# wanmeihuali/taichi_3d_gaussian_splatting

Hardware: NVIDIA H100
Metric: rendered Mpix/sec fwd+bwd @1080p, 1e6 Gaussians (higher is better)
Workload: dtype f32

## Files before the change

### taichi_3d_gaussian_splatting_b200/csrc/blend_bwd_transposed.cu

```cuda
#include "blend_bwd.cuh"

namespace gsb {

constexpr int TB_CHUNK = 16;
constexpr int TB_ROW = TB_CHUNK + 1;
constexpr int TB_TR_ROW = 13;

struct TbShared {
    float4 rec[2 * 3 * GSB_TILE_PIXELS];
    float4 g[8][32];
    float xg[8][32 * TB_ROW];
    float xa[8][32 * TB_ROW];
    int off[2][GSB_TILE_PIXELS];
    float4 chunk[8][3][TB_CHUNK];
    int chunk_off[8][TB_CHUNK];
    unsigned int bits[2][8][8];
    unsigned char list[8][GSB_TILE_PIXELS];
    int max_last;
};
static_assert(32 * TB_ROW >= TB_CHUNK * TB_TR_ROW, "finished rows must fit into the exchange buffer");

#ifdef GSB_HOST_EMU
static inline unsigned char *tb_dynamic_smem() { return simt_emu::dynamic_smem(); }
#else
extern __shared__ __align__(16) unsigned char gsb_tb_dynamic_smem[];
__device__ __forceinline__ unsigned char *tb_dynamic_smem() { return gsb_tb_dynamic_smem; }
#endif

#ifndef GSB_TB_P1_UNROLL
#define GSB_TB_P1_UNROLL 4
#endif
constexpr int TB_P1_UNROLL = GSB_TB_P1_UNROLL;
#ifndef GSB_TB_MIN_BLOCKS
#define GSB_TB_MIN_BLOCKS 3
#endif
__device__ __forceinline__ float keep_if_contributing(float P, int idx, int last) {
#ifdef GSB_HOST_EMU
    return ((idx < last) && (P >= 1.0f / 255.0f)) ? P : 0.0f;
#else
    float r;
    asm("{\n"
        ".reg .pred p, q;\n"
        "setp.lt.s32 q, %2, %3;\n"
        "setp.ge.and.f32 p, %1, 0f3B808081, q;\n"
        "selp.f32 %0, %1, 0f00000000, p;\n"
        "}\n"
        : "=f"(r)
        : "f"(P), "r"(idx), "r"(last));
    return r;
#endif
}

template <bool EXACT_EXP, bool STATS, bool COUNT = false>
__global__ void __launch_bounds__(GSB_TILE_PIXELS, GSB_TB_MIN_BLOCKS)
blend_backward_transposed_kernel(const BlendBwdParams p) {
    TbShared &S = *reinterpret_cast<TbShared *>(tb_dynamic_smem());
    constexpr int NV = STATS ? 11 : 9;

    const int tile = blockIdx.x;
    const int tu = tile % p.tiles_x, tv = tile / p.tiles_x;
    const int tid = threadIdx.x, lane = tid & 31, warp = tid >> 5;
    const int pu = tu * GSB_TILE_WIDTH + (warp & 1) * 8 + (lane & 7);
    const int pv = tv * GSB_TILE_HEIGHT + (warp >> 1) * 4 + (lane >> 3);
    const float px = (float)pu + 0.5f, py = (float)pv + 0.5f;
    const float tile_x0 = (float)(tu * GSB_TILE_WIDTH), tile_y0 = (float)(tv * GSB_TILE_HEIGHT);
    const size_t pix = (size_t)pv * p.W + pu;
    const int start = p.tile_start[tile];

    const int last = p.last_effective[pix];
    float T = 1.0f - p.acc_alpha[pix];
    float w0 = 0.0f, w1 = 0.0f, w2 = 0.0f;
    const float g0 = p.grad_image[3 * pix], g1 = p.grad_image[3 * pix + 1], g2 = p.grad_image[3 * pix + 2];
    float mag0 = 0.0f, mag1 = 0.0f;
    unsigned int n_visits = 0, n_pairs = 0;
    S.g[warp][lane] = make_float4(g0, g1, g2, 0.0f);

    const int ci = lane & (TB_CHUNK - 1), half = lane >> 4;
    const float pxb = tile_x0 + (float)((warp & 1) * 8) + 0.5f;
    const float pyb = tile_y0 + (float)((warp >> 1) * 4 + 2 * half) + 0.5f;
    float *const xg = S.xg[warp], *const xa = S.xa[warp];
    const int fl_row = lane >= GSB_ACCUM_FLOATS ? 1 : 0;
    const int fl_word = lane - GSB_ACCUM_FLOATS * fl_row;
    const bool fl_ok = lane < 2 * GSB_ACCUM_FLOATS && fl_word < NV;
    const int *const fl_off = S.chunk_off[warp] + fl_row;
    const float *const fl_val = xg + fl_row * TB_TR_ROW + (fl_ok ? fl_word : 0);
    unsigned char *const list = S.list[warp];

    int warp_last = last;
#pragma unroll
    for (int d = 16; d > 0; d >>= 1) warp_last = max(warp_last, __shfl_xor_sync(0xffffffffu, warp_last, d));
    if (tid == 0) S.max_last = start;
    __syncthreads();
    if (lane == 0) atomicMax(&S.max_last, warp_last);
    __syncthreads();
    const int end = min(p.tile_end[tile], S.max_last);

    float4 *const ck0 = S.chunk[warp][0], *const ck1 = S.chunk[warp][1], *const ck2 = S.chunk[warp][2];
    int *const ck_off = S.chunk_off[warp];
    int have = 0;

    int buf = 0;
    for (int block_end = end;; block_end -= GSB_TILE_PIXELS, buf ^= 1) {
        const bool real = block_end > start;
        int count = 0;
        float4 *const s_r0 = S.rec + buf * 3 * GSB_TILE_PIXELS;
        float4 *const s_r1 = s_r0 + GSB_TILE_PIXELS, *const s_r2 = s_r0 + 2 * GSB_TILE_PIXELS;
        if (real) {
            const int block_start = max(block_end - GSB_TILE_PIXELS, start);
            {
                const int idx = block_end - 1 - tid;
                unsigned int mask = 0;
                if (idx >= block_start) {
                    const int o = __ldg(&p.sorted_vals[idx]);
                    const float4 *rec = p.records + 3 * (size_t)o;
                    const float4 r0 = __ldg(rec), r1 = __ldg(rec + 1);
                    if (EXACT_EXP) {
                        s_r0[tid] = r0;
                        s_r1[tid] = r1;
                    } else {
                        float4 f0, f1;
                        fast_planes(r0, r1, f0, f1);
                        s_r0[tid] = f0;
                        s_r1[tid] = f1;
                    }
                    s_r2[tid] = __ldg(rec + 2);
                    S.off[buf][tid] = o;
                    mask = splat_patch_mask(r0.x, r0.y, r0.z, r0.w, r1.x, r1.y * r1.z, tile_x0, tile_y0);
                }
#pragma unroll
                for (int w = 0; w < 8; ++w) {
                    const unsigned int bits = __ballot_sync(0xffffffffu, (mask >> w) & 1u);
                    if (lane == 0) S.bits[buf][w][warp] = bits;
                }
            }
            __syncthreads();
            if (tid == 0) GSB_EMU_COUNT(EC_BATCHES, 1);
            if (block_start < warp_last) {
                const int skip = block_end - warp_last;
#pragma unroll
                for (int k = 0; k < 8; ++k) {
                    unsigned int bits = S.bits[buf][warp][k];
                    const int lo = skip - 32 * k;
                    if (lo >= 32) bits = 0u;
                    else if (lo > 0) bits &= ~((1u << lo) - 1u);
                    if ((bits >> lane) & 1u)
                        list[count + __popc(bits & ((1u << lane) - 1u))] = (unsigned char)(k * 32 + lane);
                    count += __popc(bits);
                }
                __syncwarp();
            }
        }

        int pos = 0;
#pragma unroll 1
        do {
            if (pos < count) {
                const int take = min(TB_CHUNK - have, count - pos);
                if (lane < take) {
                    const int j = list[pos + lane], slot = have + lane;
                    ck0[slot] = s_r0[j];
                    ck1[slot] = s_r1[j];
                    float4 r2 = s_r2[j];
                    r2.w = __int_as_float(block_end - 1 - j);
                    ck2[slot] = r2;
                    ck_off[slot] = S.off[buf][j];
                }
                have += take;
                pos += take;
                __syncwarp();
            }
            if (have == TB_CHUNK || (!real && have > 0)) {
                const int n = have;
                have = 0;
                if (COUNT) n_visits += (lane == 0) ? (unsigned int)n : 0u;
                if (lane == 0) {
                    GSB_EMU_COUNT(EC_TB_SPLATS, n);
                    GSB_EMU_COUNT(EC_TB_CHUNKS, 1);
                }
#pragma unroll TB_P1_UNROLL
                for (int i = 0; i < n; ++i) {
                    const float4 r0 = ck0[i];
                    const float4 r1 = ck1[i];
                    const float4 r2 = ck2[i];
                    const int idx = __float_as_int(r2.w);
                    const float d0 = px - r0.x, d1 = py - r0.y;
                    float G, aT;
                    if (EXACT_EXP) {
                        const float q0 = r0.z * d0 + r0.w * d1;
                        const float q1 = r0.w * d0 + r1.x * d1;
                        const float gp = expf(-0.5f * (d0 * q0 + d1 * q1)) * r1.y;
                        const float prod_alpha = gp * r1.z;
                        const bool contributes = (idx < last) && (prod_alpha >= 1.0f / 255.0f);
                        const float alpha = fminf(prod_alpha, 0.99f);
                        const float inv = 1.0f / (1.0f - alpha);
                        const float Tn = T * inv;
                        aT = contributes ? alpha * Tn : 0.0f;
                        const float a_grad = contributes ? (r2.x * Tn - w0 * inv) * g0 + (r2.y * Tn - w1 * inv) * g1 +
                                                               (r2.z * Tn - w2 * inv) * g2
                                                         : 0.0f;
                        T = contributes ? Tn : T;
                        w0 = fmaf(r2.x, aT, w0);
                        w1 = fmaf(r2.y, aT, w1);
                        w2 = fmaf(r2.z, aT, w2);
                        G = a_grad * r1.z * gp;
                        if (STATS) {
                            mag0 += fabsf(G * q0);
                            mag1 += fabsf(G * q1);
                        }
                    } else {
                        float P = fast_alpha(d0, d1, r0.z, r0.w, r1.x, r1.y);
                        P = keep_if_contributing(P, idx, last);
                        const float alpha = fminf(P, 0.99f);
                        const float inv = rcp_approx(1.0f - alpha);
                        T *= inv;
                        aT = alpha * T;
                        const float cg = fmaf(r2.z, g2, fmaf(r2.y, g1, r2.x * g0));
                        const float a_grad = fmaf(cg, T, -(w0 * inv));
                        w0 = fmaf(cg, aT, w0);
                        G = a_grad * P;
                        if (STATS) {
                            const float q0 = (-2.0f / GSB_L2E) * fmaf(r0.z, d0, 0.5f * r0.w * d1);
                            const float q1 = (-2.0f / GSB_L2E) * fmaf(0.5f * r0.w, d0, r1.x * d1);
                            mag0 += fabsf(G * q0);
                            mag1 += fabsf(G * q1);
                        }
                    }
                    if (COUNT) n_pairs += aT > 0.0f ? 1u : 0u;
                    xg[lane * TB_ROW + i] = G;
                    xa[lane * TB_ROW + i] = aT;
                }
                __syncwarp();

                const bool active = ci < n;
                float4 s0 = ck0[active ? ci : 0];
                float4 s1 = ck1[active ? ci : 0];
                if (!EXACT_EXP) {
                    s0.z *= -2.0f / GSB_L2E;
                    s0.w *= -1.0f / GSB_L2E;
                    s1.x *= -2.0f / GSB_L2E;
                }
                const float dx0 = pxb - s0.x;
                float acc[11];
#pragma unroll
                for (int k = 0; k < 11; ++k) acc[k] = 0.0f;
                unsigned int nz = 0u;
#pragma unroll
                for (int row = 0; row < 2; ++row) {
                    const float d1 = (pyb + (float)row) - s0.y;
                    float q0 = s0.z * dx0 + s0.w * d1;
                    float q1 = s0.w * dx0 + s1.x * d1;
#pragma unroll
                    for (int k = 0; k < 8; ++k) {
                        const int pp = 8 * row + k + 16 * half;
                        const float G = xg[pp * TB_ROW + ci], aT = xa[pp * TB_ROW + ci];
                        const float4 gp = S.g[warp][pp];
                        const float vs0 = G * q0, vs1 = G * q1;
                        acc[0] += vs0;
                        acc[1] += vs1;
                        acc[2] = fmaf(vs0, q0, acc[2]);
                        acc[3] = fmaf(vs0, q1, acc[3]);
                        acc[4] = fmaf(vs1, q1, acc[4]);
                        acc[5] = fmaf(aT, gp.x, acc[5]);
                        acc[6] = fmaf(aT, gp.y, acc[6]);
                        acc[7] = fmaf(aT, gp.z, acc[7]);
                        acc[8] += G;
                        if (STATS) {
                            const float m2 = vs0 * vs0 + vs1 * vs1;
                            acc[9] += EXACT_EXP ? sqrtf(m2) : sqrt_approx(m2);
                            acc[10] += aT > 0.0f ? 1.0f : 0.0f;
                        }
                        nz |= __float_as_uint(aT);
                        q0 += s0.z;
                        q1 += s0.w;
                    }
                }
#pragma unroll
                for (int k = 0; k < NV; ++k) acc[k] += __shfl_xor_sync(0xffffffffu, acc[k], 16);
                nz |= __shfl_xor_sync(0xffffffffu, nz, 16);
                acc[8] *= EXACT_EXP ? (1.0f - s1.z) : s1.z;
                __syncwarp();
                if (lane < TB_CHUNK) {
                    if (!(active && nz != 0u)) ck_off[ci] = -1;
                    else GSB_EMU_COUNT(EC_TB_ROWS, 1);
#pragma unroll
                    for (int k = 0; k < NV; ++k) xg[ci * TB_TR_ROW + k] = acc[k];
                }
                __syncwarp();
#pragma unroll
                for (int step = 0; step < TB_CHUNK / 2; ++step) {
                    const int o = fl_off[2 * step];
                    const float v = fl_val[2 * step * TB_TR_ROW];
                    if (fl_ok && o >= 0) atomicAdd(p.accum + (size_t)o * GSB_ACCUM_FLOATS + fl_word, v);
                }
                __syncwarp();
            }
        } while (pos < count);
        if (!real) break;
    }
    if (STATS) {
        p.mag_image[2 * pix] = mag0;
        p.mag_image[2 * pix + 1] = mag1;
    }
    if (COUNT) {
#pragma unroll
        for (int d = 16; d > 0; d >>= 1) {
            n_visits += __shfl_xor_sync(0xffffffffu, n_visits, d);
            n_pairs += __shfl_xor_sync(0xffffffffu, n_pairs, d);
        }
        if (lane == 0) {
            atomicAdd(p.work_counters, (unsigned long long)n_visits);
            atomicAdd(p.work_counters + 1, (unsigned long long)n_pairs);
        }
    }
}

#ifndef GSB_HOST_EMU
template <bool EXACT_EXP, bool STATS>
static int launch_tb(const BlendBwdParams &p, int tiles, cudaStream_t stream) {
    static bool configured = false;
    if (!configured) {
        GSB_CUDA_CHECK(cudaFuncSetAttribute(blend_backward_transposed_kernel<EXACT_EXP, STATS>,
                                            cudaFuncAttributeMaxDynamicSharedMemorySize, (int)sizeof(TbShared)));
        configured = true;
    }
    blend_backward_transposed_kernel<EXACT_EXP, STATS><<<tiles, GSB_TILE_PIXELS, sizeof(TbShared), stream>>>(p);
    GSB_CUDA_CHECK(cudaGetLastError());
    return GSB_OK;
}

int launch_blend_backward_transposed(const BlendBwdParams &p, int tiles, bool exact_exp, bool stats,
                                     cudaStream_t stream) {
    if (exact_exp) return stats ? launch_tb<true, true>(p, tiles, stream) : launch_tb<true, false>(p, tiles, stream);
    return stats ? launch_tb<false, true>(p, tiles, stream) : launch_tb<false, false>(p, tiles, stream);
}

int launch_blend_backward_count(const BlendBwdParams &p, int tiles, cudaStream_t stream) {
    GSB_CUDA_CHECK(cudaFuncSetAttribute(blend_backward_transposed_kernel<false, false, true>,
                                        cudaFuncAttributeMaxDynamicSharedMemorySize, (int)sizeof(TbShared)));
    blend_backward_transposed_kernel<false, false, true><<<tiles, GSB_TILE_PIXELS, sizeof(TbShared), stream>>>(p);
    GSB_CUDA_CHECK(cudaGetLastError());
    return GSB_OK;
}
#endif

}
```

Measured before the change: 1153.

## Factor phase-2 moments per row, interleave G/aT, and use float4 vector atomics

Phase 2 now accumulates per-row moments (sum G, sum k*G, sum k^2*G) of the Gaussian weight and reconstructs the five geometric gradient terms algebraically per row, instead of doing per-pixel q0/q1 products. G and aT are stored interleaved as float2, and the Gaussian id is packed into r2.w so the separate offset array goes away. Per-warp shared state is regrouped into a struct. The final flush uses float4 atomicAdd (sm_90 vector reduction) over three 16-byte segments per Gaussian instead of scalar atomics. The chunk size becomes configurable (8 or 16), and phase 1 is unrolled in fixed groups for full chunks. The moment-based reconstruction changes floating-point rounding slightly, and the 12-float writes add one unused zero per row.

```diff
diff --git a/taichi_3d_gaussian_splatting_b200/csrc/blend_bwd_transposed.cu b/taichi_3d_gaussian_splatting_b200/csrc/blend_bwd_transposed.cu
--- a/taichi_3d_gaussian_splatting_b200/csrc/blend_bwd_transposed.cu
+++ b/taichi_3d_gaussian_splatting_b200/csrc/blend_bwd_transposed.cu
@@ -2,23 +2,39 @@
 
 namespace gsb {
 
-constexpr int TB_CHUNK = 16;
+#ifndef GSB_TB_CHUNK
+#define GSB_TB_CHUNK 16
+#endif
+#ifndef GSB_TB_MIN_BLOCKS
+#if GSB_TB_CHUNK == 8
+#define GSB_TB_MIN_BLOCKS 4
+#else
+#define GSB_TB_MIN_BLOCKS 3
+#endif
+#endif
+constexpr int TB_CHUNK = GSB_TB_CHUNK;
+static_assert(TB_CHUNK == 8 || TB_CHUNK == 16, "a phase-2 lane takes whole rows of the 8 x 4 patch");
+constexpr int TB_ROWS = TB_CHUNK / 8;
 constexpr int TB_ROW = TB_CHUNK + 1;
-constexpr int TB_TR_ROW = 13;
-
+
+struct TbWarp {
+    float4 g[32];
+    float4 chunk[3][TB_CHUNK];
+    float2 x[32 * TB_ROW];
+    int chunk_off[TB_CHUNK];
+    unsigned char list[GSB_TILE_PIXELS];
+};
 struct TbShared {
     float4 rec[2 * 3 * GSB_TILE_PIXELS];
-    float4 g[8][32];
-    float xg[8][32 * TB_ROW];
-    float xa[8][32 * TB_ROW];
-    int off[2][GSB_TILE_PIXELS];
-    float4 chunk[8][3][TB_CHUNK];
-    int chunk_off[8][TB_CHUNK];
+    TbWarp w[8];
     unsigned int bits[2][8][8];
-    unsigned char list[8][GSB_TILE_PIXELS];
+    float2 origin;
     int max_last;
 };
-static_assert(32 * TB_ROW >= TB_CHUNK * TB_TR_ROW, "finished rows must fit into the exchange buffer");
+static_assert(2 * 32 * TB_ROW >= TB_CHUNK * GSB_ACCUM_FLOATS && GSB_ACCUM_FLOATS == 12,
+              "the finished rows (3 float4 each) must fit into the exchange buffer");
+static_assert(GSB_TB_MIN_BLOCKS * (sizeof(TbShared) + 1024) <= 228 * 1024,
+              "the shared-memory image does not allow GSB_TB_MIN_BLOCKS CTAs per SM");
 
 #ifdef GSB_HOST_EMU
 static inline unsigned char *tb_dynamic_smem() { return simt_emu::dynamic_smem(); }
@@ -31,9 +47,17 @@
 #define GSB_TB_P1_UNROLL 4
 #endif
 constexpr int TB_P1_UNROLL = GSB_TB_P1_UNROLL;
-#ifndef GSB_TB_MIN_BLOCKS
-#define GSB_TB_MIN_BLOCKS 3
-#endif
+static_assert(TB_CHUNK % TB_P1_UNROLL == 0, "a full chunk is a whole number of phase-1 groups");
+__device__ __forceinline__ void red_add_f32x4(float *addr, const float4 v) {
+#ifdef GSB_HOST_EMU
+    atomicAdd(addr, v.x);
+    atomicAdd(addr + 1, v.y);
+    atomicAdd(addr + 2, v.z);
+    atomicAdd(addr + 3, v.w);
+#else
+    atomicAdd(reinterpret_cast<float4 *>(addr), v);
+#endif
+}
 __device__ __forceinline__ float keep_if_contributing(float P, int idx, int last) {
 #ifdef GSB_HOST_EMU
     return ((idx < last) && (P >= 1.0f / 255.0f)) ? P : 0.0f;
@@ -63,7 +87,6 @@
     const int pu = tu * GSB_TILE_WIDTH + (warp & 1) * 8 + (lane & 7);
     const int pv = tv * GSB_TILE_HEIGHT + (warp >> 1) * 4 + (lane >> 3);
     const float px = (float)pu + 0.5f, py = (float)pv + 0.5f;
-    const float tile_x0 = (float)(tu * GSB_TILE_WIDTH), tile_y0 = (float)(tv * GSB_TILE_HEIGHT);
     const size_t pix = (size_t)pv * p.W + pu;
     const int start = p.tile_start[tile];
 
@@ -73,30 +96,28 @@
     const float g0 = p.grad_image[3 * pix], g1 = p.grad_image[3 * pix + 1], g2 = p.grad_image[3 * pix + 2];
     float mag0 = 0.0f, mag1 = 0.0f;
     unsigned int n_visits = 0, n_pairs = 0;
-    S.g[warp][lane] = make_float4(g0, g1, g2, 0.0f);
-
-    const int ci = lane & (TB_CHUNK - 1), half = lane >> 4;
-    const float pxb = tile_x0 + (float)((warp & 1) * 8) + 0.5f;
-    const float pyb = tile_y0 + (float)((warp >> 1) * 4 + 2 * half) + 0.5f;
-    float *const xg = S.xg[warp], *const xa = S.xa[warp];
-    const int fl_row = lane >= GSB_ACCUM_FLOATS ? 1 : 0;
-    const int fl_word = lane - GSB_ACCUM_FLOATS * fl_row;
-    const bool fl_ok = lane < 2 * GSB_ACCUM_FLOATS && fl_word < NV;
-    const int *const fl_off = S.chunk_off[warp] + fl_row;
-    const float *const fl_val = xg + fl_row * TB_TR_ROW + (fl_ok ? fl_word : 0);
-    unsigned char *const list = S.list[warp];
+    TbWarp &Wp = S.w[warp];
+    Wp.g[lane] = make_float4(g0, g1, g2, 0.0f);
+
+    const int ci = lane % TB_CHUNK, row0 = (lane / TB_CHUNK) * TB_ROWS;
+    float2 *const x = Wp.x;
+    float4 *const fin = reinterpret_cast<float4 *>(x);
+    unsigned char *const list = Wp.list;
 
     int warp_last = last;
 #pragma unroll
     for (int d = 16; d > 0; d >>= 1) warp_last = max(warp_last, __shfl_xor_sync(0xffffffffu, warp_last, d));
-    if (tid == 0) S.max_last = start;
+    if (tid == 0) {
+        S.max_last = start;
+        S.origin = make_float2((float)(tu * GSB_TILE_WIDTH), (float)(tv * GSB_TILE_HEIGHT));
+    }
     __syncthreads();
     if (lane == 0) atomicMax(&S.max_last, warp_last);
     __syncthreads();
     const int end = min(p.tile_end[tile], S.max_last);
 
-    float4 *const ck0 = S.chunk[warp][0], *const ck1 = S.chunk[warp][1], *const ck2 = S.chunk[warp][2];
-    int *const ck_off = S.chunk_off[warp];
+    float4 *const ck0 = Wp.chunk[0], *const ck1 = Wp.chunk[1], *const ck2 = Wp.chunk[2];
+    int *const ck_off = Wp.chunk_off;
     int have = 0;
 
     int buf = 0;
@@ -123,9 +144,10 @@
                         s_r0[tid] = f0;
                         s_r1[tid] = f1;
                     }
-                    s_r2[tid] = __ldg(rec + 2);
-                    S.off[buf][tid] = o;
-                    mask = splat_patch_mask(r0.x, r0.y, r0.z, r0.w, r1.x, r1.y * r1.z, tile_x0, tile_y0);
+                    float4 r2 = __ldg(rec + 2);
+                    r2.w = __int_as_float(o);
+                    s_r2[tid] = r2;
+                    mask = splat_patch_mask(r0.x, r0.y, r0.z, r0.w, r1.x, r1.y * r1.z, S.origin.x, S.origin.y);
                 }
 #pragma unroll
                 for (int w = 0; w < 8; ++w) {
@@ -161,9 +183,9 @@
                     ck0[slot] = s_r0[j];
                     ck1[slot] = s_r1[j];
                     float4 r2 = s_r2[j];
+                    ck_off[slot] = __float_as_int(r2.w);
                     r2.w = __int_as_float(block_end - 1 - j);
                     ck2[slot] = r2;
-                    ck_off[slot] = S.off[buf][j];
                 }
                 have += take;
                 pos += take;
@@ -177,8 +199,7 @@
                     GSB_EMU_COUNT(EC_TB_SPLATS, n);
                     GSB_EMU_COUNT(EC_TB_CHUNKS, 1);
                 }
-#pragma unroll TB_P1_UNROLL
-                for (int i = 0; i < n; ++i) {
+                const auto p1 = [&](const int i) -> float2 {
                     const float4 r0 = ck0[i];
                     const float4 r1 = ck1[i];
                     const float4 r2 = ck2[i];
@@ -226,8 +247,20 @@
                         }
                     }
                     if (COUNT) n_pairs += aT > 0.0f ? 1u : 0u;
-                    xg[lane * TB_ROW + i] = G;
-                    xa[lane * TB_ROW + i] = aT;
+                    return make_float2(G, aT);
+                };
+                if (n == TB_CHUNK) {
+#pragma unroll 1
+                    for (int i0 = 0; i0 < TB_CHUNK; i0 += TB_P1_UNROLL) {
+                        float2 ex[TB_P1_UNROLL];
+#pragma unroll
+                        for (int u = 0; u < TB_P1_UNROLL; ++u) ex[u] = p1(i0 + u);
+#pragma unroll
+                        for (int u = 0; u < TB_P1_UNROLL; ++u) x[lane * TB_ROW + i0 + u] = ex[u];
+                    }
+                } else {
+#pragma unroll 1
+                    for (int i = 0; i < n; ++i) x[lane * TB_ROW + i] = p1(i);
                 }
                 __syncwarp();
 
@@ -239,58 +272,73 @@
                     s0.w *= -1.0f / GSB_L2E;
                     s1.x *= -2.0f / GSB_L2E;
                 }
-                const float dx0 = pxb - s0.x;
+                const float ca = s0.z, cb = s0.w, cc = s1.x;
+                const float2 org = S.origin;
+                const float pxc = org.x + (float)((warp & 1) * 8) + 4.0f;
+                const float pyb = org.y + (float)((warp >> 1) * 4 + row0) + 0.5f;
+                const float dxc = pxc - s0.x;
                 float acc[11];
 #pragma unroll
                 for (int k = 0; k < 11; ++k) acc[k] = 0.0f;
                 unsigned int nz = 0u;
 #pragma unroll
-                for (int row = 0; row < 2; ++row) {
+                for (int row = 0; row < TB_ROWS; ++row) {
                     const float d1 = (pyb + (float)row) - s0.y;
-                    float q0 = s0.z * dx0 + s0.w * d1;
-                    float q1 = s0.w * dx0 + s1.x * d1;
+                    const float q0r = fmaf(ca, dxc, cb * d1);
+                    const float q1r = fmaf(cb, dxc, cc * d1);
+                    float m0 = 0.0f, m1 = 0.0f, m2 = 0.0f;
 #pragma unroll
                     for (int k = 0; k < 8; ++k) {
-                        const int pp = 8 * row + k + 16 * half;
-                        const float G = xg[pp * TB_ROW + ci], aT = xa[pp * TB_ROW + ci];
-                        const float4 gp = S.g[warp][pp];
-                        const float vs0 = G * q0, vs1 = G * q1;
-                        acc[0] += vs0;
-                        acc[1] += vs1;
-                        acc[2] = fmaf(vs0, q0, acc[2]);
-                        acc[3] = fmaf(vs0, q1, acc[3]);
-                        acc[4] = fmaf(vs1, q1, acc[4]);
-                        acc[5] = fmaf(aT, gp.x, acc[5]);
-                        acc[6] = fmaf(aT, gp.y, acc[6]);
-                        acc[7] = fmaf(aT, gp.z, acc[7]);
-                        acc[8] += G;
+                        const float kc = (float)k - 3.5f;
+                        const int pp = 8 * (row0 + row) + k;
+                        const float2 ga = x[pp * TB_ROW + ci];
+                        const float4 gp = Wp.g[pp];
+                        m0 += ga.x;
+                        m1 = fmaf(kc, ga.x, m1);
+                        m2 = fmaf(kc * kc, ga.x, m2);
+                        acc[5] = fmaf(ga.y, gp.x, acc[5]);
+                        acc[6] = fmaf(ga.y, gp.y, acc[6]);
+                        acc[7] = fmaf(ga.y, gp.z, acc[7]);
                         if (STATS) {
-                            const float m2 = vs0 * vs0 + vs1 * vs1;
-                            acc[9] += EXACT_EXP ? sqrtf(m2) : sqrt_approx(m2);
-                            acc[10] += aT > 0.0f ? 1.0f : 0.0f;
+                            const float vs0 = ga.x * fmaf(ca, kc, q0r), vs1 = ga.x * fmaf(cb, kc, q1r);
+                            const float mm = vs0 * vs0 + vs1 * vs1;
+                            acc[9] += EXACT_EXP ? sqrtf(mm) : sqrt_approx(mm);
+                            acc[10] += ga.y > 0.0f ? 1.0f : 0.0f;
                         }
-                        nz |= __float_as_uint(aT);
-                        q0 += s0.z;
-                        q1 += s0.w;
-                    }
-                }
-#pragma unroll
-                for (int k = 0; k < NV; ++k) acc[k] += __shfl_xor_sync(0xffffffffu, acc[k], 16);
-                nz |= __shfl_xor_sync(0xffffffffu, nz, 16);
+                        nz |= __float_as_uint(ga.y);
+                    }
+                    const float t0 = fmaf(ca, m1, q0r * m0), t1 = fmaf(cb, m1, q1r * m0);
+                    const float u0 = fmaf(ca, m2, q0r * m1), u1 = fmaf(cb, m2, q1r * m1);
+                    acc[0] += t0;
+                    acc[1] += t1;
+                    acc[2] += fmaf(ca, u0, q0r * t0);
+                    acc[3] += fmaf(cb, u0, q1r * t0);
+                    acc[4] += fmaf(cb, u1, q1r * t1);
+                    acc[8] += m0;
+                }
+#pragma unroll
+                for (int d = TB_CHUNK; d < 32; d *= 2) {
+#pragma unroll
+                    for (int k = 0; k < NV; ++k) acc[k] += __shfl_xor_sync(0xffffffffu, acc[k], d);
+                    nz |= __shfl_xor_sync(0xffffffffu, nz, d);
+                }
                 acc[8] *= EXACT_EXP ? (1.0f - s1.z) : s1.z;
                 __syncwarp();
                 if (lane < TB_CHUNK) {
                     if (!(active && nz != 0u)) ck_off[ci] = -1;
                     else GSB_EMU_COUNT(EC_TB_ROWS, 1);
-#pragma unroll
-                    for (int k = 0; k < NV; ++k) xg[ci * TB_TR_ROW + k] = acc[k];
-                }
-                __syncwarp();
-#pragma unroll
-                for (int step = 0; step < TB_CHUNK / 2; ++step) {
-                    const int o = fl_off[2 * step];
-                    const float v = fl_val[2 * step * TB_TR_ROW];
-                    if (fl_ok && o >= 0) atomicAdd(p.accum + (size_t)o * GSB_ACCUM_FLOATS + fl_word, v);
+                    fin[3 * ci] = make_float4(acc[0], acc[1], acc[2], acc[3]);
+                    fin[3 * ci + 1] = make_float4(acc[4], acc[5], acc[6], acc[7]);
+                    fin[3 * ci + 2] = make_float4(acc[8], STATS ? acc[9] : 0.0f, STATS ? acc[10] : 0.0f, 0.0f);
+                }
+                __syncwarp();
+#pragma unroll
+                for (int e0 = 0; e0 < 3 * TB_CHUNK; e0 += 32) {
+                    const int e = e0 + lane, row = e / 3;
+                    if (e < 3 * TB_CHUNK) {
+                        const int o = ck_off[row];
+                        if (o >= 0) red_add_f32x4(p.accum + (size_t)o * GSB_ACCUM_FLOATS + 4 * (e - 3 * row), fin[e]);
+                    }
                 }
                 __syncwarp();
             }
```

After: 1246, median of 6. 1.08x the previous value.
